# markchil/gptools

Measured on AMD Instinct MI355X. Metric: K-build+Cholesky GFLOP/s (% fp64 MFMA peak) and LML evals/sec, N=8192, higher is better.
Workload: dtype f64

## Files before the change

gptools_amd/csrc/gemm.hip:

```cpp
#include "common.hpp"

#define GM_BK 16
#define GPT_TRY_RC(expr) do { int rc_ = (expr); if (rc_ != GPT_OK) return rc_; } while (0)

typedef const __attribute__((address_space(1))) void *gptr_t;
typedef __attribute__((address_space(3))) void *lptr_t;

__device__ __forceinline__ int64_t xcd_remap(int64_t pid, int64_t nwg)
{
    const int64_t q = nwg >> 3, r = nwg & 7;
    const int64_t xcd = pid & 7, local = pid >> 3;
    const int64_t base = (xcd < r) ? xcd * (q + 1) : r * (q + 1) + (xcd - r) * q;
    return base + local;
}

__device__ __forceinline__ void tile_decode(int64_t id, int tri, int64_t ntn, int64_t *ti, int64_t *tj)
{
    if (tri) {
        const int64_t ntri = ntn * (ntn + 1) / 2;
        if (id < ntri) {
            int64_t t = (int64_t)((sqrt(8.0 * (double)id + 1.0) - 1.0) * 0.5);
            while (t * (t + 1) / 2 > id) t--;
            while ((t + 1) * (t + 2) / 2 <= id) t++;
            *ti = t;
            *tj = id - t * (t + 1) / 2;
        } else {
            const int64_t r = id - ntri;
            *ti = ntn + r / ntn;
            *tj = r % ntn;
        }
    } else {
        *ti = id / ntn;
        *tj = id % ntn;
    }
}

template <int R>
__device__ __forceinline__ void stage_ptrs(const double *M, int64_t ld, int64_t r0, int64_t lim, int wave, int lane,
                                           const double *(&src)[R / 32])
{
#pragma unroll
    for (int qq = 0; qq < R / 32; qq++) {
        const int q = wave * (R / 32) + qq;
        const int row = q * 8 + (lane >> 3);
        const int c = (lane & 7) ^ ((row >> 1) & 7);
        int64_t gr = r0 + row;
        if (gr >= lim) gr = lim - 1;
        src[qq] = M + gr * ld + c * 2;
    }
}

__device__ __forceinline__ void glds16(const double *gsrc, unsigned lds_byte_addr)
{
    unsigned keep;
    asm volatile("s_mov_b32 %0, m0\n\ts_mov_b32 m0, %2\n\ts_nop 0\n\tglobal_load_lds_dwordx4 %1, off\n\ts_mov_b32 m0, %0"
                 : "=&s"(keep)
                 : "v"(gsrc), "s"(lds_byte_addr)
                 : "memory");
}

__device__ __forceinline__ void dma_wait() { asm volatile("s_waitcnt vmcnt(0)" ::: "memory"); }

__device__ __forceinline__ unsigned lds_addr(const void *p)
{
    return (unsigned)(uintptr_t)(__attribute__((address_space(3))) const void *)p;
}

template <int R>
__device__ __forceinline__ void stage_issue(const double *const (&src)[R / 32], int64_t koff, unsigned tile_lds, int wave)
{
#pragma unroll
    for (int qq = 0; qq < R / 32; qq++) {
        const int q = wave * (R / 32) + qq;
        glds16(src[qq] + koff, tile_lds + (unsigned)(q * 8 * GM_BK * sizeof(double)));
    }
}

template <int RM, int RN>
__device__ __forceinline__ void mma_ktile(const double *tA, const double *tB, int arow0, int brow0, int fr, int fk,
                                          f64x4 (&acc)[RM][RN])
{
    const int sw = (fr >> 1) & 7;
#pragma unroll
    for (int t = 0; t < GM_BK / 8; t++) {
        const int p = ((fk + 4 * t) ^ sw) * 2;
        f64x2 af[RM], bf[RN];
#pragma unroll
        for (int i = 0; i < RM; i++) af[i] = *reinterpret_cast<const f64x2 *>(tA + (arow0 + i * 16 + fr) * GM_BK + p);
#pragma unroll
        for (int j = 0; j < RN; j++) bf[j] = *reinterpret_cast<const f64x2 *>(tB + (brow0 + j * 16 + fr) * GM_BK + p);
#pragma unroll
        for (int u = 0; u < 2; u++)
#pragma unroll
            for (int i = 0; i < RM; i++)
#pragma unroll
                for (int j = 0; j < RN; j++)
                    acc[i][j] = __builtin_amdgcn_mfma_f64_16x16x4f64(af[i][u], bf[j][u], acc[i][j], 0, 0, 0);
    }
}

#ifdef GPT_GEMM_STAMPS
__device__ long long *g_gemm_stamps;
#define GM_STAMP(i) do { if (threadIdx.x == 0) g_gemm_stamps[(long long)blockIdx.x * 8 + (i)] = (long long)wall_clock64(); } while (0)
#else
#define GM_STAMP(i) do { } while (0)
#endif

#ifdef GPT_GEMM_C_NT
#define GM_LOADC(p) __builtin_nontemporal_load(p)
#define GM_STOREC(v, p) __builtin_nontemporal_store((v), (p))
#elif defined(GPT_GEMM_C_NTLOAD)
#define GM_LOADC(p) __builtin_nontemporal_load(p)
#define GM_STOREC(v, p) (*(p) = (v))
#else
#define GM_LOADC(p) (*(p))
#define GM_STOREC(v, p) (*(p) = (v))
#endif
template <int BM, int BN, int NSTAGE>
__device__ __forceinline__ void gemm_tile_body(
    int64_t row0, int64_t col0, int64_t tj, double *sA, double *sB,
    int64_t m, int64_t n, int64_t k, double alpha, const double *__restrict__ A, int64_t lda,
    const double *__restrict__ B, int64_t ldb, double beta, double *__restrict__ C, int64_t ldc,
    int64_t seg_cols, int64_t bskip, int prio, unsigned *edge, unsigned edge_val,
    unsigned edge_total, const unsigned *wait_word, unsigned wait_val, unsigned *wait_err, int edge_cols,
    const unsigned *tail_word, unsigned tail_val, unsigned *tail_err)
{
    constexpr int WM = BM / 2, WN = BN / 2;
    constexpr int RM = WM / 16, RN = WN / 16;
    GM_STAMP(6);
    const int tid = threadIdx.x, lane = tid & 63;
    if (edge_cols > 0 && tj >= edge_cols) edge = nullptr;
    if (wait_word != nullptr) {
        if (tid == 0) edge_poll<16, false>(wait_word, wait_val, wait_err);
        __syncthreads();
    }
    const int wave = __builtin_amdgcn_readfirstlane(tid >> 6);
    const int wm = wave >> 1, wn = wave & 1;
    const int fr = lane & 15, fk = lane >> 4;

    const double *srcA[BM / 32], *srcB[BN / 32];
    stage_ptrs<BM>(A, lda, row0, m, wave, lane, srcA);
    const int64_t brow0 = seg_cols ? col0 + (col0 / seg_cols) * bskip : col0;
    stage_ptrs<BN>(B, ldb, brow0, seg_cols ? (int64_t)1 << 62 : n, wave, lane, srcB);
    const unsigned ldsA = lds_addr(sA), ldsB = lds_addr(sB);
    constexpr unsigned ABYTES = BM * GM_BK * sizeof(double), BBYTES = BN * GM_BK * sizeof(double);
    const int64_t nk = k / GM_BK;
    constexpr int PRE = NSTAGE - 1;
    constexpr int PERSTAGE = BM / 32 + BN / 32;
    f64x4 acc[RM][RN];
    const double cs = (beta != 0.0) ? beta / alpha : 0.0;
#pragma unroll
    for (int i = 0; i < RM; i++)
#pragma unroll
        for (int j = 0; j < RN; j++) {
            const int64_t col = col0 + wn * WN + j * 16 + fr;
#pragma unroll
            for (int r = 0; r < 4; r++) {
                const int64_t row = row0 + wm * WM + i * 16 + fk + 4 * r;
                acc[i][j][r] = (beta != 0.0 && row < m && col < n)
                                   ? (wait_word ? __hip_atomic_load(&C[row * ldc + col], __ATOMIC_RELAXED, __HIP_MEMORY_SCOPE_AGENT)
                                                : GM_LOADC(&C[row * ldc + col]))
                                   : 0.0;
            }
        }
    GM_STAMP(7);
#pragma unroll
    for (int t = 0; t < PRE; t++)
        if (t < nk) {
            stage_issue<BM>(srcA, (int64_t)t * GM_BK, ldsA + t * ABYTES, wave);
            stage_issue<BN>(srcB, (int64_t)t * GM_BK, ldsB + t * BBYTES, wave);
        }
#pragma unroll
    for (int i = 0; i < RM; i++)
#pragma unroll
        for (int j = 0; j < RN; j++) acc[i][j] = acc[i][j] * cs;
    GM_STAMP(4);
    if (NSTAGE == 2 || nk < PRE) dma_wait();
    else asm volatile("s_waitcnt vmcnt(%0)" ::"n"((PRE - 1) * PERSTAGE) : "memory");
    GM_STAMP(5);
    __syncthreads();
#ifndef GPT_GEMM_NOPRIO
    if (prio == 0) __builtin_amdgcn_s_setprio(0);
    else if (prio == 1) __builtin_amdgcn_s_setprio(1);
    else if (prio == 2) __builtin_amdgcn_s_setprio(2);
#endif
    GM_STAMP(1);

    for (int64_t kt = 0; kt < nk; kt++) {
        const int cur = (int)(kt % NSTAGE);
        if (kt + PRE < nk) {
            const int nxt = (int)((kt + PRE) % NSTAGE);
            stage_issue<BM>(srcA, (kt + PRE) * GM_BK, ldsA + nxt * ABYTES, wave);
            stage_issue<BN>(srcB, (kt + PRE) * GM_BK, ldsB + nxt * BBYTES, wave);
        }
        mma_ktile<RM, RN>(sA + cur * (BM * GM_BK), sB + cur * (BN * GM_BK), wm * WM, wn * WN, fr, fk, acc);
        if (NSTAGE == 2 || kt + PRE >= nk) dma_wait();
        else asm volatile("s_waitcnt vmcnt(%0)" ::"n"((PRE - 1) * PERSTAGE) : "memory");
        __syncthreads();
    }
    GM_STAMP(2);

#pragma unroll
    for (int i = 0; i < RM; i++)
#pragma unroll
        for (int j = 0; j < RN; j++) {
            const int64_t col = col0 + wn * WN + j * 16 + fr;
#pragma unroll
            for (int r = 0; r < 4; r++) {
                const int64_t row = row0 + wm * WM + i * 16 + fk + 4 * r;
                if (row < m && col < n) {
                    if (edge) __hip_atomic_store(&C[row * ldc + col], alpha * acc[i][j][r], __ATOMIC_RELAXED, __HIP_MEMORY_SCOPE_AGENT);
                    else GM_STOREC(alpha * acc[i][j][r], &C[row * ldc + col]);
                }
            }
        }
    GM_STAMP(3);
    if (edge) edge_signal(edge, edge_val, edge_total);
    if (tail_word != nullptr && blockIdx.x == gridDim.x - 1 && blockIdx.y == 0 && tid == 0) edge_poll<16, false>(tail_word, tail_val, tail_err);
}

template <int BM, int BN, int WPS, int NSTAGE>
__global__ __launch_bounds__(256, WPS) void gemm_nt_kernel(
    int64_t m, int64_t n, int64_t k, double alpha, const double *__restrict__ A, int64_t lda,
    const double *__restrict__ B, int64_t ldb, double beta, double *__restrict__ C, int64_t ldc,
    int tri, int64_t ntm, int64_t ntn, int64_t nwg, const int2 *__restrict__ order, int64_t seg_cols, int64_t bskip, int prio, unsigned *edge, unsigned edge_val,
    unsigned edge_total, const unsigned *wait_word, unsigned wait_val, unsigned *wait_err, int edge_cols, int64_t bstride,
    const unsigned *tail_word, unsigned tail_val, unsigned *tail_err, int64_t bstride_b, int64_t bstride_c)
{
    A += (int64_t)blockIdx.y * bstride;
    B += (int64_t)blockIdx.y * bstride_b;
    C += (int64_t)blockIdx.y * bstride_c;
    __shared__ __attribute__((aligned(16))) double sA[NSTAGE * BM * GM_BK];
    __shared__ __attribute__((aligned(16))) double sB[NSTAGE * BN * GM_BK];

    GM_STAMP(0);
#ifndef GPT_GEMM_NOPRIO
    __builtin_amdgcn_s_setprio(3);
#endif
    int64_t ti, tj;
    if (order != nullptr) {
        const int2 t = order[blockIdx.x];
        if (t.x < 0) {
            if (tail_word != nullptr && blockIdx.x == gridDim.x - 1 && threadIdx.x == 0) edge_poll<16, false>(tail_word, tail_val, tail_err);
            return;
        }
        ti = t.x;
        tj = t.y;
    } else {
        tile_decode(xcd_remap(blockIdx.x, nwg), tri, ntn, &ti, &tj);
    }
    gemm_tile_body<BM, BN, NSTAGE>(ti * BM, tj * BN, tj, sA, sB, m, n, k, alpha, A, lda, B, ldb, beta, C, ldc, seg_cols, bskip, prio, edge,
                                   edge_val, edge_total, wait_word, wait_val, wait_err, edge_cols, tail_word, tail_val, tail_err);
}

#include <algorithm>
#include <cstdio>
#include <cstdlib>
#include <mutex>
#include <vector>
struct TileOrder {
    int64_t ntm, ntn;
    int tri, dev;
    int64_t seg_t, rss_t;
    int64_t g_off, g_num, g_den, g_base;
    int2 *d_tab;
    int64_t grid;
    int64_t ntiles;
    int64_t edge_cols, nedge;
    uint64_t last_use;
    bool pinned;
};
static std::vector<TileOrder> g_orders;
static std::mutex g_orders_mu;
static uint64_t g_orders_tick = 0;

struct GridStair { int64_t off = 0, num = 0, den = 1, base = 0; };
static inline bool tile_needed(int tri, int64_t i, int64_t j, int64_t seg_t, int64_t rss_t, const GridStair &g = GridStair())
{
    if (tri == 1) return j <= i;
    if (tri == 2) {
        const int64_t q = j / seg_t;
        return i >= q * rss_t + (j - q * seg_t);
    }
    if (tri == 3) {
        const int64_t q = j / seg_t, v = g.off + q * g.num;
        const int64_t i0 = ((v + g.den - 1) / g.den - g.base) * seg_t;
        if (i < i0) return false;
        if (v % g.den == 0 && i < i0 + seg_t) return (i - i0) >= (j - q * seg_t);
        return true;
    }
    return true;
}

static int tile_order(int64_t ntm, int64_t ntn, int tri, const int2 **tab, int64_t *grid, int64_t seg_t = 0,
                      int64_t rss_t = 0, int64_t *ntiles = nullptr, int64_t edge_cols = 0, int64_t *nedge = nullptr,
                      const GridStair &gs = GridStair(), hipStream_t st = nullptr)
{
    static int sgm = 0, sgn = 0, mode = 0;
    if (sgm == 0) {
        sgm = 64, sgn = 8, mode = 1;
        if (const char *e = getenv("GPT_TILE_ORDER")) {
            int a = 0, b = 0, c = 0;
            if (sscanf(e, "%d,%d,%d", &a, &b, &c) >= 2 && a > 0 && b > 0) sgm = a, sgn = b, mode = c;
        }
    }
    int dev = 0;
    GPT_HIP_CHECK(hipGetDevice(&dev));
    bool capturing = false;
    if (st != nullptr) {
        hipStreamCaptureStatus cs = hipStreamCaptureStatusNone;
        if (hipStreamIsCapturing(st, &cs) == hipSuccess) capturing = (cs != hipStreamCaptureStatusNone);
        else (void)hipGetLastError();
    }
    std::lock_guard<std::mutex> lk(g_orders_mu);
    for (auto &o : g_orders)
        if (o.ntm == ntm && o.ntn == ntn && o.tri == tri && o.dev == dev && o.seg_t == seg_t && o.rss_t == rss_t && o.edge_cols == edge_cols &&
            o.g_off == gs.off && o.g_num == gs.num && o.g_den == gs.den && o.g_base == gs.base) {
            o.last_use = ++g_orders_tick;
            o.pinned = o.pinned || capturing;
            *tab = o.d_tab;
            *grid = o.grid;
            if (ntiles) *ntiles = o.ntiles;
            if (nedge) *nedge = o.nedge;
            return GPT_OK;
        }
    if (g_orders.size() >= 1024 && !capturing) {
        if (hipDeviceSynchronize() == hipSuccess) {
            std::vector<uint64_t> ticks;
            for (const auto &o : g_orders)
                if (!o.pinned) ticks.push_back(o.last_use);
            if (ticks.size() >= 2) {
                std::nth_element(ticks.begin(), ticks.begin() + ticks.size() / 2, ticks.end());
                const uint64_t cut = ticks[ticks.size() / 2];
                std::vector<TileOrder> keep;
                for (const auto &o : g_orders) {
                    if (!o.pinned && o.last_use < cut) (void)hipFree(o.d_tab);
                    else keep.push_back(o);
                }
                g_orders.swap(keep);
            }
        } else {
            (void)hipGetLastError();
        }
    }
    std::vector<std::vector<int2>> per(8);
    std::vector<int2> seq, sequ;
    const int64_t sm = (ntm + sgm - 1) / sgm, sn = (ntn + sgn - 1) / sgn;
    int64_t sidx = 0;
    for (int64_t si = 0; si < sm; si++)
        for (int64_t sj = 0; sj < sn; sj++) {
            std::vector<int2> &dst = (mode || edge_cols > 0) ? seq : per[sidx % 8];
            bool any = false;
            for (int64_t i = si * sgm; i < (si + 1) * sgm && i < ntm; i++)
                for (int64_t j = sj * sgn; j < (sj + 1) * sgn && j < ntn; j++) {
                    if (!tile_needed(tri, i, j, seg_t, rss_t, gs)) continue;
                    (j < edge_cols ? sequ : dst).push_back(make_int2((int)i, (int)j));
                    any = true;
                }
            if (any) sidx++;
        }
    if (mode || edge_cols > 0) {
        for (const std::vector<int2> *sq : {&sequ, &seq}) {
            const size_t T = sq->size(), q = T / 8, r = T % 8;
            size_t at = 0;
            for (int x = 0; x < 8; x++) {
                const size_t len = q + ((size_t)x < r ? 1 : 0);
                per[x].insert(per[x].end(), sq->begin() + at, sq->begin() + at + len);
                at += len;
            }
        }
    }
    size_t mx = 0;
    for (auto &v : per) mx = v.size() > mx ? v.size() : mx;
    std::vector<int2> flat(mx * 8, make_int2(-1, -1));
    for (int x = 0; x < 8; x++)
        for (size_t l = 0; l < per[x].size(); l++) flat[l * 8 + x] = per[x][l];
    TileOrder o;
    o.ntm = ntm;
    o.ntn = ntn;
    o.tri = tri;
    o.dev = dev;
    o.seg_t = seg_t;
    o.rss_t = rss_t;
    o.g_off = gs.off;
    o.g_num = gs.num;
    o.g_den = gs.den;
    o.g_base = gs.base;
    o.edge_cols = edge_cols;
    o.nedge = (int64_t)sequ.size();
    o.grid = (int64_t)flat.size();
    o.ntiles = 0;
    for (auto &v : per) o.ntiles += (int64_t)v.size();
    o.d_tab = nullptr;
    GPT_HIP_CHECK(hipMalloc(&o.d_tab, flat.size() * sizeof(int2)));
    {
        hipStream_t up = nullptr;
        GPT_HIP_CHECK(hipStreamCreateWithFlags(&up, hipStreamNonBlocking));
        hipError_t e1 = hipMemcpyAsync(o.d_tab, flat.data(), flat.size() * sizeof(int2), hipMemcpyHostToDevice, up);
        hipError_t e2 = hipStreamSynchronize(up);
        hipStreamDestroy(up);
        if (e1 != hipSuccess || e2 != hipSuccess) (void)hipFree(o.d_tab);
        GPT_HIP_CHECK(e1);
        GPT_HIP_CHECK(e2);
    }
    o.last_use = ++g_orders_tick;
    o.pinned = capturing;
    g_orders.push_back(o);
    *tab = o.d_tab;
    *grid = o.grid;
    if (ntiles) *ntiles = o.ntiles;
    if (nedge) *nedge = o.nedge;
    return GPT_OK;
}

template <int BM, int BN, int WPS, int NSTAGE>
static int gemm_launch_t(hipStream_t st, int64_t m, int64_t n, int64_t k, double alpha, const double *A,
                         int64_t lda, const double *B, int64_t ldb, double beta, double *C, int64_t ldc, int tri,
                         int lds_pad, hipEvent_t ev0 = nullptr, hipEvent_t ev1 = nullptr, int64_t seg_cols = 0,
                         int64_t bskip = 0, int64_t row_step = 0, int prio = 0, EdgeSig edge = EdgeSig(),
                         EdgeSig wait = EdgeSig(), int64_t edge_cols_elems = 0, int64_t nbatch = 1, int64_t bstride = 0,
                         EdgeSig tail = EdgeSig(), int64_t bstride_b = -1, int64_t bstride_c = -1, const GridStair &gs = GridStair())
{
    if (bstride_b < 0) bstride_b = bstride;
    if (bstride_c < 0) bstride_c = bstride;
    const int64_t ntm = (m + BM - 1) / BM, ntn = (n + BN - 1) / BN;
    int64_t nwg = (tri == 1) ? ntn * (ntn + 1) / 2 + (ntm - ntn) * ntn : ntm * ntn;
    int64_t nreal = nwg;
    int64_t nedge = 0;
    const int2 *order = nullptr;
    if (tri == 2) {
        int64_t grid = 0;
        GPT_TRY_RC(tile_order(ntm, ntn, 2, &order, &grid, seg_cols / BN, row_step / BM, &nreal, 0, nullptr, GridStair(), st));
        nwg = grid;
    } else if (tri == 3) {
        int64_t grid = 0;
        GPT_TRY_RC(tile_order(ntm, ntn, 3, &order, &grid, seg_cols / BN, 0, &nreal, 0, nullptr, gs, st));
        nwg = grid;
    } else if (nwg >= 512) {
        int64_t grid = 0;
        GPT_TRY_RC(tile_order(ntm, ntn, tri, &order, &grid, 0, 0, &nreal, edge_cols_elems / BN, &nedge, GridStair(), st));
        nwg = grid;
    }
    if (edge_cols_elems > 0 && (order == nullptr || !edge.word || nedge <= 0)) {
        gpt_set_error("gemm_nt: a partial edge flag needs a launch large enough for an order table");
        return GPT_E_ARG;
    }
    if (nwg <= 0) return GPT_OK;
    const size_t dyn = (BM == 64) ? (size_t)lds_pad : 0;
    if (ev0 || ev1)
        hipExtLaunchKernelGGL((gemm_nt_kernel<BM, BN, WPS, NSTAGE>), dim3((unsigned)nwg, (unsigned)nbatch), dim3(256), dyn, st, ev0, ev1, 0,
                              m, n, k, alpha, A, lda, B, ldb, beta, C, ldc, tri, ntm, ntn, nwg, order, seg_cols, bskip, prio, edge.word, edge.value,
                              (unsigned)(edge_cols_elems > 0 ? nedge : nreal), wait.word, wait.value, wait.err, (int)(edge_cols_elems / BN), bstride,
                              tail.word, tail.value, tail.err, bstride_b, bstride_c);
    else
        hipLaunchKernelGGL((gemm_nt_kernel<BM, BN, WPS, NSTAGE>), dim3((unsigned)nwg, (unsigned)nbatch), dim3(256), dyn, st, m, n, k, alpha,
                           A, lda, B, ldb, beta, C, ldc, tri, ntm, ntn, nwg, order, seg_cols, bskip, prio, edge.word, edge.value,
                              (unsigned)(edge_cols_elems > 0 ? nedge : nreal), wait.word, wait.value, wait.err, (int)(edge_cols_elems / BN), bstride,
                              tail.word, tail.value, tail.err, bstride_b, bstride_c);
    GPT_LAUNCH_CHECK();
    return GPT_OK;
}

int gemm_small_threshold()
{
    static int small_below = -1;
    if (small_below < 0) {
        small_below = 512;
        if (const char *e = getenv("GPT_GEMM_SMALL")) small_below = atoi(e);
    }
    return small_below;
}

int launch_gemm_nt(hipStream_t st, int64_t m, int64_t n, int64_t k, double alpha, const double *A, int64_t lda,
                   const double *B, int64_t ldb, double beta, double *C, int64_t ldc, int tri, int force_tile, int lds_pad,
                   hipEvent_t ev0, hipEvent_t ev1, int prio, EdgeSig edge, EdgeSig wait, int64_t edge_cols, int64_t nbatch,
                   int64_t bstride, EdgeSig tail, int64_t bstride_b, int64_t bstride_c)
{
    gpt_jitter(st);
    if (m <= 0 || n <= 0) {
        if (edge.word) {
            gpt_set_error("gemm_nt: an empty launch cannot raise an edge flag");
            return GPT_E_ARG;
        }
        return GPT_OK;
    }
    if (alpha == 0.0) {
        gpt_set_error("gemm_nt: alpha must be non-zero");
        return GPT_E_ARG;
    }
    if (k <= 0 || (k % GM_BK) != 0 || (lda & 1) || (ldb & 1)) {
        gpt_set_error("gemm_nt: k must be a positive multiple of %d and lda/ldb even (k=%lld)", GM_BK, (long long)k);
        return GPT_E_ARG;
    }
    if (((uintptr_t)A & 15) || ((uintptr_t)B & 15)) {
        gpt_set_error("gemm_nt: A and B must be 16-byte aligned");
        return GPT_E_ARG;
    }
    if (tri && m < n) {
        gpt_set_error("gemm_nt: tri requires m >= n");
        return GPT_E_ARG;
    }
    if (nbatch > 1 && (force_tile != 0 || edge.word || wait.word || edge_cols || ev0 || ev1)) {
        gpt_set_error("gemm_nt: batched launches take the default tiles, no edges and no events");
        return GPT_E_ARG;
    }
    int tile = force_tile;
    if (tile == 0) {
        tile = 64;
        const int small_below = gemm_small_threshold();
        const int64_t nt64 = ((m + 63) / 64) * ((n + 63) / 64);
        if (nt64 < small_below && !ev0 && edge_cols == 0) tile = 32;
    }
    if (tile == 32) {
        static int stages = -1;
        if (stages < 0) {
            stages = 0;
            if (const char *e = getenv("GPT_GEMM_SMALL_STAGES")) stages = atoi(e);
        }
        if ((stages == 4 && k >= 64) || (stages == 0 && k >= 256))
            return gemm_launch_t<32, 32, 2, 4>(st, m, n, k, alpha, A, lda, B, ldb, beta, C, ldc, tri, 0, ev0, ev1, 0, 0, 0, prio, edge, wait, 0, nbatch, bstride, tail, bstride_b, bstride_c);
        return gemm_launch_t<32, 32, 2, 2>(st, m, n, k, alpha, A, lda, B, ldb, beta, C, ldc, tri, 0, ev0, ev1, 0, 0, 0, prio, edge, wait, 0, nbatch, bstride, tail, bstride_b, bstride_c);
    }
    if ((edge.word || wait.word || edge_cols || tail.word) && tile != 64) {
        gpt_set_error("gemm_nt: edge flags exist for the 64x64 / 32x32 kernels only");
        return GPT_E_ARG;
    }
    if (tile != 64) {
        gpt_set_error("gemm_nt: option tile takes 0 (by size), 32 or 64");
        return GPT_E_ARG;
    }
    return gemm_launch_t<64, 64, 2, 2>(st, m, n, k, alpha, A, lda, B, ldb, beta, C, ldc, tri, lds_pad, ev0, ev1, 0, 0, 0, prio, edge, wait, edge_cols,
                                       nbatch, bstride, tail, bstride_b, bstride_c);
}

int launch_gemm_nt_stair(hipStream_t st, int64_t m, int64_t nseg, int64_t seg_cols, int64_t k, double alpha,
                         const double *A, int64_t lda, const double *B, int64_t ldb, int64_t b_stride, int64_t row_step,
                         double beta, double *C, int64_t ldc, int lds_pad, hipEvent_t ev0, hipEvent_t ev1)
{
    gpt_jitter(st);
    if (m <= 0 || nseg <= 0) return GPT_OK;
    if (alpha == 0.0 || k <= 0 || (k % GM_BK) != 0 || (lda & 1) || (ldb & 1) || ((uintptr_t)A & 15) ||
        ((uintptr_t)B & 15) || seg_cols <= 0 || (seg_cols % 64) || (row_step % 64) || b_stride < seg_cols) {
        gpt_set_error("gemm_nt_stair: bad arguments (k multiple of %d, seg_cols / row_step multiples of 64, 16-byte "
                      "aligned operands)", GM_BK);
        return GPT_E_ARG;
    }
    return gemm_launch_t<64, 64, 2, 2>(st, m, nseg * seg_cols, k, alpha, A, lda, B, ldb, beta, C, ldc, 2, lds_pad, ev0,
                                       ev1, seg_cols, b_stride - seg_cols, row_step);
}

int launch_gemm_nt_gridstair(hipStream_t st, int64_t m, int64_t nseg, int64_t seg_cols, int64_t k, double alpha, const double *A,
                             int64_t lda, const double *B, int64_t ldb, int64_t off, int64_t num, int64_t den, int64_t base,
                             double beta, double *C, int64_t ldc, int lds_pad, hipEvent_t ev0, hipEvent_t ev1)
{
    gpt_jitter(st);
    if (m <= 0 || nseg <= 0) return GPT_OK;
    if (alpha == 0.0 || k <= 0 || (k % GM_BK) != 0 || (lda & 1) || (ldb & 1) || ((uintptr_t)A & 15) || ((uintptr_t)B & 15) ||
        seg_cols <= 0 || (seg_cols % 64) || num <= 0 || den <= 0 || off <= -den) {
        gpt_set_error("gemm_nt_gridstair: bad arguments (k multiple of %d, seg_cols a multiple of 64, num, den > 0, 16-byte "
                      "aligned operands)", GM_BK);
        return GPT_E_ARG;
    }
    GridStair gs;
    gs.off = off;
    gs.num = num;
    gs.den = den;
    gs.base = base;
    return gemm_launch_t<64, 64, 2, 2>(st, m, nseg * seg_cols, k, alpha, A, lda, B, ldb, beta, C, ldc, 3, lds_pad, ev0, ev1, seg_cols, 0,
                                       0, 0, EdgeSig(), EdgeSig(), 0, 1, 0, EdgeSig(), -1, -1, gs);
}
```

Measured before the change: 39460.

## Add inline-asm global-to-LDS DMA body with scalar base and 32-bit offsets

Adds a second GEMM mainloop variant that issues global_load_lds_dwordx4 through inline assembly. It uses one scalar base pointer per operand plus precomputed 32-bit per-lane offsets instead of per-lane 64-bit pointers, and sets m0 directly. The k-loop is unrolled by NSTAGE so stage indices are compile-time constants. A GPT_GEMM_BODY environment switch picks the variant, defaulting to the new body for 32x32 tiles only when offsets fit in 32 bits. The aim is to cut VGPR pressure and per-iteration address arithmetic, at the cost of hand-written asm with manual hazard NOPs and m0 save/restore.

Result: no change. 39850 (median of 6 runs) (+1.0%).

```diff
diff --git a/gptools_amd/csrc/gemm.hip b/gptools_amd/csrc/gemm.hip
--- a/gptools_amd/csrc/gemm.hip
+++ b/gptools_amd/csrc/gemm.hip
@@ -76,6 +76,51 @@
     }
 }
 
+template <int R>
+__device__ __forceinline__ void stage_offs(int64_t ld, int64_t r0, int64_t lim, int wave, int lane, unsigned (&off)[R / 32])
+{
+#pragma unroll
+    for (int qq = 0; qq < R / 32; qq++) {
+        const int q = wave * (R / 32) + qq;
+        const int row = q * 8 + (lane >> 3);
+        const int c = (lane & 7) ^ ((row >> 1) & 7);
+        int64_t gr = r0 + row;
+        if (gr >= lim) gr = lim - 1;
+        off[qq] = (unsigned)(((gr - r0) * ld + c * 2) * (int64_t)sizeof(double));
+    }
+}
+
+#define GM_DMA64 \
+    "s_mov_b32 %0, m0\n\t"                                                                    \
+    "s_mov_b32 m0, %5\n\ts_nop 0\n\tglobal_load_lds_dwordx4 %1, %7\n\t"                          \
+    "s_add_u32 m0, %5, 0x400\n\ts_nop 0\n\tglobal_load_lds_dwordx4 %2, %7\n\t"                   \
+    "s_mov_b32 m0, %6\n\ts_nop 0\n\tglobal_load_lds_dwordx4 %3, %8\n\t"                          \
+    "s_add_u32 m0, %6, 0x400\n\ts_nop 0\n\tglobal_load_lds_dwordx4 %4, %8\n\t"                   \
+    "s_mov_b32 m0, %0"
+#define GM_DMA32 \
+    "s_mov_b32 %0, m0\n\t"                                                                    \
+    "s_mov_b32 m0, %3\n\ts_nop 0\n\tglobal_load_lds_dwordx4 %1, %5\n\t"                          \
+    "s_mov_b32 m0, %4\n\ts_nop 0\n\tglobal_load_lds_dwordx4 %2, %6\n\t"                          \
+    "s_mov_b32 m0, %0"
+template <int BM, int BN, bool FIRST>
+__device__ __forceinline__ void stage_dma(const double *gA, const unsigned (&oa)[BM / 32], unsigned la,
+                                          const double *gB, const unsigned (&ob)[BN / 32], unsigned lb)
+{
+    static_assert(BM == BN && (BM == 64 || BM == 32), "stage_dma: 32x32 or 64x64 tiles");
+    unsigned keep;
+    const gptr_t sa = (gptr_t)gA, sb = (gptr_t)gB;
+    if constexpr (BM == 64 && FIRST)
+        asm volatile("s_nop 4\n\t" GM_DMA64 : "=&s"(keep) : "v"(oa[0]), "v"(oa[1]), "v"(ob[0]), "v"(ob[1]), "s"(la), "s"(lb),
+                     "s"(sa), "s"(sb) : "memory", "scc");
+    else if constexpr (BM == 64)
+        asm volatile(GM_DMA64 : "=&s"(keep) : "v"(oa[0]), "v"(oa[1]), "v"(ob[0]), "v"(ob[1]), "s"(la), "s"(lb), "s"(sa), "s"(sb)
+                     : "memory", "scc");
+    else if constexpr (FIRST)
+        asm volatile("s_nop 4\n\t" GM_DMA32 : "=&s"(keep) : "v"(oa[0]), "v"(ob[0]), "s"(la), "s"(lb), "s"(sa), "s"(sb) : "memory");
+    else
+        asm volatile(GM_DMA32 : "=&s"(keep) : "v"(oa[0]), "v"(ob[0]), "s"(la), "s"(lb), "s"(sa), "s"(sb) : "memory");
+}
+
 template <int RM, int RN>
 __device__ __forceinline__ void mma_ktile(const double *tA, const double *tB, int arow0, int brow0, int fr, int fk,
                                           f64x4 (&acc)[RM][RN])
@@ -116,7 +161,7 @@
 #define GM_LOADC(p) (*(p))
 #define GM_STOREC(v, p) (*(p) = (v))
 #endif
-template <int BM, int BN, int NSTAGE>
+template <int BM, int BN, int NSTAGE, int BODY>
 __device__ __forceinline__ void gemm_tile_body(
     int64_t row0, int64_t col0, int64_t tj, double *sA, double *sB,
     int64_t m, int64_t n, int64_t k, double alpha, const double *__restrict__ A, int64_t lda,
@@ -138,12 +183,22 @@
     const int wm = wave >> 1, wn = wave & 1;
     const int fr = lane & 15, fk = lane >> 4;
 
-    const double *srcA[BM / 32], *srcB[BN / 32];
-    stage_ptrs<BM>(A, lda, row0, m, wave, lane, srcA);
     const int64_t brow0 = seg_cols ? col0 + (col0 / seg_cols) * bskip : col0;
-    stage_ptrs<BN>(B, ldb, brow0, seg_cols ? (int64_t)1 << 62 : n, wave, lane, srcB);
+    const int64_t blim = seg_cols ? (int64_t)1 << 62 : n;
     const unsigned ldsA = lds_addr(sA), ldsB = lds_addr(sB);
     constexpr unsigned ABYTES = BM * GM_BK * sizeof(double), BBYTES = BN * GM_BK * sizeof(double);
+    const double *srcA[BM / 32], *srcB[BN / 32];
+    unsigned offA[BM / 32], offB[BN / 32];
+    const double *gA = A + row0 * lda, *gB = B + brow0 * ldb;
+    const unsigned ldsAw = ldsA + (unsigned)(wave * (BM / 32) * 8 * GM_BK * sizeof(double));
+    const unsigned ldsBw = ldsB + (unsigned)(wave * (BN / 32) * 8 * GM_BK * sizeof(double));
+    if constexpr (BODY == 0) {
+        stage_ptrs<BM>(A, lda, row0, m, wave, lane, srcA);
+        stage_ptrs<BN>(B, ldb, brow0, blim, wave, lane, srcB);
+    } else {
+        stage_offs<BM>(lda, row0, m, wave, lane, offA);
+        stage_offs<BN>(ldb, brow0, blim, wave, lane, offB);
+    }
     const int64_t nk = k / GM_BK;
     constexpr int PRE = NSTAGE - 1;
     constexpr int PERSTAGE = BM / 32 + BN / 32;
@@ -167,8 +222,12 @@
 #pragma unroll
     for (int t = 0; t < PRE; t++)
         if (t < nk) {
-            stage_issue<BM>(srcA, (int64_t)t * GM_BK, ldsA + t * ABYTES, wave);
-            stage_issue<BN>(srcB, (int64_t)t * GM_BK, ldsB + t * BBYTES, wave);
+            if constexpr (BODY == 0) {
+                stage_issue<BM>(srcA, (int64_t)t * GM_BK, ldsA + t * ABYTES, wave);
+                stage_issue<BN>(srcB, (int64_t)t * GM_BK, ldsB + t * BBYTES, wave);
+            } else {
+                stage_dma<BM, BN, true>(gA + t * GM_BK, offA, ldsAw + t * ABYTES, gB + t * GM_BK, offB, ldsBw + t * BBYTES);
+            }
         }
 #pragma unroll
     for (int i = 0; i < RM; i++)
@@ -186,17 +245,37 @@
 #endif
     GM_STAMP(1);
 
-    for (int64_t kt = 0; kt < nk; kt++) {
-        const int cur = (int)(kt % NSTAGE);
-        if (kt + PRE < nk) {
-            const int nxt = (int)((kt + PRE) % NSTAGE);
-            stage_issue<BM>(srcA, (kt + PRE) * GM_BK, ldsA + nxt * ABYTES, wave);
-            stage_issue<BN>(srcB, (kt + PRE) * GM_BK, ldsB + nxt * BBYTES, wave);
-        }
-        mma_ktile<RM, RN>(sA + cur * (BM * GM_BK), sB + cur * (BN * GM_BK), wm * WM, wn * WN, fr, fk, acc);
-        if (NSTAGE == 2 || kt + PRE >= nk) dma_wait();
-        else asm volatile("s_waitcnt vmcnt(%0)" ::"n"((PRE - 1) * PERSTAGE) : "memory");
-        __syncthreads();
+    if constexpr (BODY == 0) {
+        for (int64_t kt = 0; kt < nk; kt++) {
+            const int cur = (int)(kt % NSTAGE);
+            if (kt + PRE < nk) {
+                const int nxt = (int)((kt + PRE) % NSTAGE);
+                stage_issue<BM>(srcA, (kt + PRE) * GM_BK, ldsA + nxt * ABYTES, wave);
+                stage_issue<BN>(srcB, (kt + PRE) * GM_BK, ldsB + nxt * BBYTES, wave);
+            }
+            mma_ktile<RM, RN>(sA + cur * (BM * GM_BK), sB + cur * (BN * GM_BK), wm * WM, wn * WN, fr, fk, acc);
+            if (NSTAGE == 2 || kt + PRE >= nk) dma_wait();
+            else asm volatile("s_waitcnt vmcnt(%0)" ::"n"((PRE - 1) * PERSTAGE) : "memory");
+            __syncthreads();
+        }
+    } else {
+        const int nki = (int)nk;
+        for (int kb = 0; kb < nki; kb += NSTAGE) {
+#pragma unroll
+            for (int cur = 0; cur < NSTAGE; cur++) {
+                const int kt = kb + cur;
+                if (kt >= nki) break;
+                if (kt + PRE < nki) {
+                    const int nxt = (cur + PRE) % NSTAGE;
+                    stage_dma<BM, BN, false>(gA + (int64_t)(kt + PRE) * GM_BK, offA, ldsAw + nxt * ABYTES,
+                                             gB + (int64_t)(kt + PRE) * GM_BK, offB, ldsBw + nxt * BBYTES);
+                }
+                mma_ktile<RM, RN>(sA + cur * (BM * GM_BK), sB + cur * (BN * GM_BK), wm * WM, wn * WN, fr, fk, acc);
+                if (NSTAGE == 2 || kt + PRE >= nki) dma_wait();
+                else asm volatile("s_waitcnt vmcnt(%0)" ::"n"((PRE - 1) * PERSTAGE) : "memory");
+                __syncthreads();
+            }
+        }
     }
     GM_STAMP(2);
 
@@ -219,7 +298,7 @@
     if (tail_word != nullptr && blockIdx.x == gridDim.x - 1 && blockIdx.y == 0 && tid == 0) edge_poll<16, false>(tail_word, tail_val, tail_err);
 }
 
-template <int BM, int BN, int WPS, int NSTAGE>
+template <int BM, int BN, int WPS, int NSTAGE, int BODY>
 __global__ __launch_bounds__(256, WPS) void gemm_nt_kernel(
     int64_t m, int64_t n, int64_t k, double alpha, const double *__restrict__ A, int64_t lda,
     const double *__restrict__ B, int64_t ldb, double beta, double *__restrict__ C, int64_t ldc,
@@ -249,7 +328,7 @@
     } else {
         tile_decode(xcd_remap(blockIdx.x, nwg), tri, ntn, &ti, &tj);
     }
-    gemm_tile_body<BM, BN, NSTAGE>(ti * BM, tj * BN, tj, sA, sB, m, n, k, alpha, A, lda, B, ldb, beta, C, ldc, seg_cols, bskip, prio, edge,
+    gemm_tile_body<BM, BN, NSTAGE, BODY>(ti * BM, tj * BN, tj, sA, sB, m, n, k, alpha, A, lda, B, ldb, beta, C, ldc, seg_cols, bskip, prio, edge,
                                    edge_val, edge_total, wait_word, wait_val, wait_err, edge_cols, tail_word, tail_val, tail_err);
 }
 
@@ -413,6 +492,17 @@
     return GPT_OK;
 }
 
+static int gemm_body()
+{
+    static int body = -1;
+    if (body < 0) {
+        body = 3;
+        if (const char *e = getenv("GPT_GEMM_BODY")) body = atoi(e);
+        if (body < 0 || body > 3) body = 3;
+    }
+    return body;
+}
+
 template <int BM, int BN, int WPS, int NSTAGE>
 static int gemm_launch_t(hipStream_t st, int64_t m, int64_t n, int64_t k, double alpha, const double *A,
                          int64_t lda, const double *B, int64_t ldb, double beta, double *C, int64_t ldc, int tri,
@@ -447,13 +537,17 @@
     }
     if (nwg <= 0) return GPT_OK;
     const size_t dyn = (BM == 64) ? (size_t)lds_pad : 0;
+    const int64_t lim32 = (int64_t)1 << 31;
+    const int mode = gemm_body();
+    const bool body1 = (mode == 1 || (mode == 2 && BM == 64) || (mode == 3 && BM == 32)) && (BM - 1) * lda * 8 + 128 < lim32 && (BN - 1) * ldb * 8 + 128 < lim32;
+    auto kern = body1 ? gemm_nt_kernel<BM, BN, WPS, NSTAGE, 1> : gemm_nt_kernel<BM, BN, WPS, NSTAGE, 0>;
     if (ev0 || ev1)
-        hipExtLaunchKernelGGL((gemm_nt_kernel<BM, BN, WPS, NSTAGE>), dim3((unsigned)nwg, (unsigned)nbatch), dim3(256), dyn, st, ev0, ev1, 0,
+        hipExtLaunchKernelGGL(kern, dim3((unsigned)nwg, (unsigned)nbatch), dim3(256), dyn, st, ev0, ev1, 0,
                               m, n, k, alpha, A, lda, B, ldb, beta, C, ldc, tri, ntm, ntn, nwg, order, seg_cols, bskip, prio, edge.word, edge.value,
                               (unsigned)(edge_cols_elems > 0 ? nedge : nreal), wait.word, wait.value, wait.err, (int)(edge_cols_elems / BN), bstride,
                               tail.word, tail.value, tail.err, bstride_b, bstride_c);
     else
-        hipLaunchKernelGGL((gemm_nt_kernel<BM, BN, WPS, NSTAGE>), dim3((unsigned)nwg, (unsigned)nbatch), dim3(256), dyn, st, m, n, k, alpha,
+        hipLaunchKernelGGL(kern, dim3((unsigned)nwg, (unsigned)nbatch), dim3(256), dyn, st, m, n, k, alpha,
                            A, lda, B, ldb, beta, C, ldc, tri, ntm, ntn, nwg, order, seg_cols, bskip, prio, edge.word, edge.value,
                               (unsigned)(edge_cols_elems > 0 ? nedge : nreal), wait.word, wait.value, wait.err, (int)(edge_cols_elems / BN), bstride,
                               tail.word, tail.value, tail.err, bstride_b, bstride_c);
```
